# nubot-nudt/MDGAT-matcher

Hardware: AMD Instinct MI355X
Metric: keypoint-pairs/sec (higher is better)
Workload: dtype f32 (products as 3 split-f16 MFMAs, fp32 accumulate)

## Files before the change

mdgat_matcher_amd/csrc/sinkhorn.hip:

```cpp
#include "common.hpp"
#include <atomic>
#include <cstdlib>

namespace {

constexpr float NEG_BIG = -1.0e30f;

struct SkArgs {
    const float* scores;
    const float* alpha_dev;
    float alpha_host;
    float* Z;
    int N, M, iters;
    const unsigned* only_if;
    unsigned* status_fallback;
    const unsigned* pair_flags;
    const int* cnt0;
    const int* cnt1;
};

__device__ __forceinline__ float wave_max(float v) {
#pragma unroll
    for (int o = 32; o > 0; o >>= 1) v = fmaxf(v, __shfl_xor(v, o, 64));
    return v;
}
__device__ __forceinline__ float wave_sum(float v) {
#pragma unroll
    for (int o = 32; o > 0; o >>= 1) v += __shfl_xor(v, o, 64);
    return v;
}
__device__ __forceinline__ float ex2(float x) { return __builtin_amdgcn_exp2f(x); }
__device__ __forceinline__ float lg2(float x) { return __builtin_amdgcn_logf(x); }

__device__ __forceinline__ float wave_lse2(const float* x, int n, float extra, int lane) {
    float m = extra;
    for (int i = lane; i < n; i += 64) m = fmaxf(m, x[i]);
    m = wave_max(m);
    float s = 0.f;
    for (int i = lane; i < n; i += 64) s += ex2(x[i] - m);
    s = wave_sum(s) + ex2(extra - m);
    return m + lg2(s);
}

template <int NC, int NW, bool RAGGED = false>
__global__ __launch_bounds__(NW * 64) void sinkhorn_kernel(SkArgs a) {
    extern __shared__ __attribute__((aligned(16))) float smem[];
    const int Ns = a.N, Ms = a.M;
    int N = Ns, M = Ms;
    if constexpr (RAGGED) { N = __builtin_amdgcn_readfirstlane(a.cnt0[blockIdx.x]); M = __builtin_amdgcn_readfirstlane(a.cnt1[blockIdx.x]); }
    const int tid = threadIdx.x, lane = tid & 63;
    const int wave = __builtin_amdgcn_readfirstlane(tid >> 6);
    if (a.only_if) {
        const bool mine = (__hip_atomic_load(a.only_if, __ATOMIC_RELAXED, __HIP_MEMORY_SCOPE_AGENT) & 1u) != 0 ||
                          (a.pair_flags && __hip_atomic_load(a.pair_flags + blockIdx.x, __ATOMIC_RELAXED, __HIP_MEMORY_SCOPE_AGENT) != 0);
        if (!mine) return;
        if (tid == 0 && a.status_fallback) __hip_atomic_store(a.status_fallback, 1u, __ATOMIC_RELAXED, __HIP_MEMORY_SCOPE_SYSTEM);
    }
    const float* S = a.scores + (size_t)blockIdx.x * Ns * Ms;
    float* Z = a.Z + (size_t)blockIdx.x * (Ns + 1) * (Ms + 1);

    float* u = smem;
    float* v = u + (N + 1);
    float* pm = v + (M + 1);
    float* ps = pm + NW * M;

    const float alpha = (a.alpha_dev ? *a.alpha_dev : a.alpha_host) * MDGAT_LOG2E;
    const float norm = -logf((float)(N + M));
    const float lmu = norm * MDGAT_LOG2E;
    const float lmuN = (logf((float)M) + norm) * MDGAT_LOG2E;
    const float lnu = lmu;
    const float lnuM = (logf((float)N) + norm) * MDGAT_LOG2E;

    for (int i = tid; i <= N; i += NW * 64) u[i] = 0.f;
    for (int j = tid; j <= M; j += NW * 64) v[j] = 0.f;
    __syncthreads();

    for (int it = 0; it < a.iters; ++it) {
        float vr[NC];
#pragma unroll
        for (int c = 0; c < NC; ++c) {
            const int j = c * 64 + lane;
            vr[c] = j < M ? v[j] : 0.f;
        }
        const float bM = alpha + v[M];
        if (wave == NW - 1) {
            const float lse = alpha + wave_lse2(v, M, v[M], lane);
            if (lane == 0) u[N] = lmuN - lse;
        }
        float cm[NC], cs[NC];
#pragma unroll
        for (int c = 0; c < NC; ++c) { cm[c] = NEG_BIG; cs[c] = 0.f; }

        for (int i = wave; i < N; i += NW) {
            const float* row = S + (size_t)i * Ms;
            float s[NC];
#pragma unroll
            for (int c = 0; c < NC; ++c) {
                const int j = c * 64 + lane;
                s[c] = j < M ? row[j] * MDGAT_LOG2E : NEG_BIG;
            }
            float m = bM;
#pragma unroll
            for (int c = 0; c < NC; ++c) m = fmaxf(m, s[c] + vr[c]);
            m = wave_max(m);
            float e = 0.f;
#pragma unroll
            for (int c = 0; c < NC; ++c) e += ex2(s[c] + vr[c] - m);
            e = wave_sum(e) + ex2(bM - m);
            const float ui = lmu - (m + lg2(e));
            if (lane == 0) u[i] = ui;
#pragma unroll
            for (int c = 0; c < NC; ++c) {
                const float w = s[c] + ui;
                const float nm = fmaxf(cm[c], w);
                cs[c] = cs[c] * ex2(cm[c] - nm) + ex2(w - nm);
                cm[c] = nm;
            }
        }
#pragma unroll
        for (int c = 0; c < NC; ++c) {
            const int j = c * 64 + lane;
            if (j < M) { pm[wave * M + j] = cm[c]; ps[wave * M + j] = cs[c]; }
        }
        __syncthreads();
        const float bN = alpha + u[N];
        for (int j = tid; j < M; j += NW * 64) {
            float m = bN;
#pragma unroll
            for (int w = 0; w < NW; ++w) m = fmaxf(m, pm[w * M + j]);
            float e = ex2(bN - m);
#pragma unroll
            for (int w = 0; w < NW; ++w) e += ps[w * M + j] * ex2(pm[w * M + j] - m);
            v[j] = lnu - (m + lg2(e));
        }
        if (wave == 0) {
            const float lse = alpha + wave_lse2(u, N, u[N], lane);
            if (lane == 0) v[M] = lnuM - lse;
        }
        __syncthreads();
    }

    const float uN = u[N], vM = v[M];
    for (int i = wave; i < N; i += NW) {
        const float ui = u[i];
        const float* row = S + (size_t)i * Ms;
        float* zr = Z + (size_t)i * (Ms + 1);
        for (int j = lane; j < M; j += 64) zr[j] = (row[j] * MDGAT_LOG2E + ui + v[j]) * MDGAT_LN2 - norm;
        if (lane == 0) zr[M] = (alpha + ui + vM) * MDGAT_LN2 - norm;
        if constexpr (RAGGED)
            for (int j = M + 1 + lane; j <= Ms; j += 64) zr[j] = 0.f;
    }
    float* zl = Z + (size_t)N * (Ms + 1);
    for (int j = tid; j <= M; j += NW * 64) zl[j] = (alpha + uN + v[j]) * MDGAT_LN2 - norm;
    if constexpr (RAGGED) {
        float* rest = zl + M + 1;
        const int nrest = (Ms - M) + (Ns - N) * (Ms + 1);
        for (int j = tid; j < nrest; j += NW * 64) rest[j] = 0.f;
    }
}


constexpr int SLOT_STRIDE = 520;

template <int CTRL, int ROW_MASK>
__device__ __forceinline__ float dpp_move(float identity, float v) {
    return __builtin_bit_cast(float, __builtin_amdgcn_update_dpp(__builtin_bit_cast(int, identity), __builtin_bit_cast(int, v),
                                                                 CTRL, ROW_MASK, 0xf, false));
}
__device__ __forceinline__ float wave_max_dpp(float v) {
    v = fmaxf(v, dpp_move<0x111, 0xf>(NEG_BIG, v));
    v = fmaxf(v, dpp_move<0x112, 0xf>(NEG_BIG, v));
    v = fmaxf(v, dpp_move<0x114, 0xf>(NEG_BIG, v));
    v = fmaxf(v, dpp_move<0x118, 0xf>(NEG_BIG, v));
    v = fmaxf(v, dpp_move<0x142, 0xa>(NEG_BIG, v));
    v = fmaxf(v, dpp_move<0x143, 0xc>(NEG_BIG, v));
    return __builtin_bit_cast(float, __builtin_amdgcn_readlane(__builtin_bit_cast(int, v), 63));
}
__device__ __forceinline__ float wave_sum_dpp(float v) {
    v += dpp_move<0x111, 0xf>(0.f, v);
    v += dpp_move<0x112, 0xf>(0.f, v);
    v += dpp_move<0x114, 0xf>(0.f, v);
    v += dpp_move<0x118, 0xf>(0.f, v);
    v += dpp_move<0x142, 0xa>(0.f, v);
    v += dpp_move<0x143, 0xc>(0.f, v);
    return __builtin_bit_cast(float, __builtin_amdgcn_readlane(__builtin_bit_cast(int, v), 63));
}

__device__ __forceinline__ void swap_halves32(float& a, float& b) { asm("s_nop 1\n\tv_permlane32_swap_b32 %0, %1\n\ts_nop 1" : "+v"(a), "+v"(b)); }
__device__ __forceinline__ void swap_rows16(float& a, float& b) { asm("s_nop 1\n\tv_permlane16_swap_b32 %0, %1\n\ts_nop 1" : "+v"(a), "+v"(b)); }
template <int CTRL, int BANK>
__device__ __forceinline__ float dpp_bank_move(float old, float v) {
    return __builtin_bit_cast(float, __builtin_amdgcn_update_dpp(__builtin_bit_cast(int, old), __builtin_bit_cast(int, v), CTRL, 0xf, BANK, false));
}
__device__ __forceinline__ float wave_sum16(float (&acc)[16], int lane) {
    float s[8];
#pragma unroll
    for (int r = 0; r < 8; ++r) { float x = acc[r], y = acc[r + 8]; swap_halves32(x, y); s[r] = x + y; }
    float t[4];
#pragma unroll
    for (int r = 0; r < 4; ++r) { float x = s[r], y = s[r + 4]; swap_rows16(x, y); t[r] = x + y; }
    const bool b3 = (lane & 8) != 0, b2 = (lane & 4) != 0;
    float v[2];
#pragma unroll
    for (int r = 0; r < 2; ++r) {
        const float keep = b3 ? t[r + 2] : t[r], give = b3 ? t[r] : t[r + 2];
        v[r] = keep + dpp_bank_move<0x128, 0xf>(0.f, give);
    }
    const float keep = b2 ? v[1] : v[0], give = b2 ? v[0] : v[1];
    float o = dpp_bank_move<0x104, 0x5>(0.f, give);
    o = dpp_bank_move<0x114, 0xa>(o, give);
    float w = keep + o;
    w += dpp_bank_move<0xb1, 0xf>(0.f, w);
    w += dpp_bank_move<0x4e, 0xf>(0.f, w);
    return __builtin_bit_cast(float, __builtin_amdgcn_ds_bpermute(16 * lane, __builtin_bit_cast(int, w)));
}

typedef __attribute__((address_space(1))) unsigned long long gu64;
#define SK_LD "sc1"

struct SksArgs {
    const float* scores;
    const float* alpha_dev;
    float alpha_host;
    float* Z;
    unsigned long long* slots;
    unsigned* error_word;
    unsigned* pair_flags;
    unsigned* range_guard;
    int B, N, M, iters, ngroups, GR, GC;
    int xcd_map;
    int ext_mode;
    int* rbest_idx;
    float* rbest_val;
    int* cbest_idx;
    float* cbest_val;
};

constexpr int SKS_THREADS = 512;
constexpr int SKS_LDS_FLOATS = 520 + 8 * 512 + 8 + 8 + 8 * 512;
constexpr int ROW_STRIDE = 136;

__device__ __forceinline__ unsigned long long xload(gu64* p, bool same_xcd) {
    if (same_xcd) {
        unsigned long long v;
        asm volatile("global_load_dwordx2 %0, %1, off " SK_LD "\n\ts_waitcnt vmcnt(0)" : "=v"(v) : "v"(p) : "memory");
        return v;
    }
    return __hip_atomic_load(p, __ATOMIC_RELAXED, __HIP_MEMORY_SCOPE_AGENT);
}
__device__ __forceinline__ void xstore(gu64* p, unsigned long long v, bool same_xcd) {
    if (same_xcd) asm volatile("global_store_dwordx2 %0, %1, off" :: "v"(p), "v"(v) : "memory");
    else __hip_atomic_store(p, v, __ATOMIC_RELAXED, __HIP_MEMORY_SCOPE_AGENT);
}

template <int NMAX>
__device__ __forceinline__ void poll_partners(gu64* base, size_t stride, int n, int self, unsigned tag, float (&vals)[NMAX],
                                              bool& failed, unsigned* error_word, bool same_xcd = false,
                                              gu64* extra = nullptr, float* extra_val = nullptr) {
    unsigned pending = ((1u << n) - 1u) & ~(1u << self);
    bool extra_pending = extra != nullptr;
    unsigned spins = 0;
    while (pending || extra_pending) {
        unsigned long long x[NMAX], xe = 0;
        if (NMAX <= 4 && same_xcd) {
#pragma unroll
            for (int p = 0; p < NMAX; ++p)
                if (pending & (1u << p)) asm volatile("global_load_dwordx2 %0, %1, off " SK_LD : "=v"(x[p]) : "v"(base + (size_t)p * stride) : "memory");
            if (extra_pending) asm volatile("global_load_dwordx2 %0, %1, off " SK_LD : "=v"(xe) : "v"(extra) : "memory");
            asm volatile("s_waitcnt vmcnt(0)" ::: "memory");
#pragma unroll
            for (int p = 0; p < NMAX; ++p)
                if (pending & (1u << p)) asm volatile("" : "+v"(x[p]));
            asm volatile("" : "+v"(xe));
        } else if (same_xcd) {
#pragma unroll
            for (int p = 0; p < NMAX; ++p) x[p] = 0;
#pragma unroll
            for (int p0 = 0; p0 < NMAX; p0 += 4) {
                if (!((pending >> p0) & 0xfu) && !(extra_pending && p0 == 0)) continue;
                unsigned long long y[4] = {0, 0, 0, 0};
#pragma unroll
                for (int u = 0; u < 4; ++u)
                    if (pending & (1u << (p0 + u))) asm volatile("global_load_dwordx2 %0, %1, off " SK_LD : "=v"(y[u]) : "v"(base + (size_t)(p0 + u) * stride) : "memory");
                if (extra_pending && p0 == 0) asm volatile("global_load_dwordx2 %0, %1, off " SK_LD : "=v"(xe) : "v"(extra) : "memory");
                asm volatile("s_waitcnt vmcnt(0)" ::: "memory");
#pragma unroll
                for (int u = 0; u < 4; ++u) {
                    asm volatile("" : "+v"(y[u]));
                    if ((pending & (1u << (p0 + u))) && (unsigned)(y[u] >> 32) == tag) {
                        vals[p0 + u] = __builtin_bit_cast(float, (unsigned)y[u]);
                        pending &= ~(1u << (p0 + u));
                    }
                }
                asm volatile("" : "+v"(xe));
            }
        } else {
#pragma unroll
            for (int p = 0; p < NMAX; ++p)
                if (pending & (1u << p)) x[p] = __hip_atomic_load(base + (size_t)p * stride, __ATOMIC_RELAXED, __HIP_MEMORY_SCOPE_AGENT);
            if (extra_pending) xe = __hip_atomic_load(extra, __ATOMIC_RELAXED, __HIP_MEMORY_SCOPE_AGENT);
        }
#pragma unroll
        for (int p = 0; p < NMAX; ++p)
            if ((pending & (1u << p)) && (unsigned)(x[p] >> 32) == tag) {
                vals[p] = __builtin_bit_cast(float, (unsigned)x[p]);
                pending &= ~(1u << p);
            }
        if (extra_pending && (unsigned)(xe >> 32) == tag) {
            *extra_val = __builtin_bit_cast(float, (unsigned)xe);
            extra_pending = false;
        }
        if (pending || extra_pending) {
            if (failed || ++spins > (1u << 22)) { failed = true; atomicOr(error_word, 1u); break; }
            __builtin_amdgcn_s_sleep(1);
        }
    }
}

template <bool TWO_D, int GMAX>
__global__ __launch_bounds__(SKS_THREADS, 2) void sinkhorn_scaling_kernel(SksArgs a) {
    constexpr int RPW = 16;
    __shared__ __attribute__((aligned(16))) float lds[SKS_LDS_FLOATS];
    float* bvec = lds;
    float* colp = lds + 520;
    float* pdust = colp + 8 * 512;
    int* flags = reinterpret_cast<int*>(pdust + 8);
    int* colpi = flags + 8;

    const int N = a.N, M = a.M, GR = a.GR, GC = TWO_D ? a.GC : 1;
    const int tid = threadIdx.x, lane = tid & 63;
    const int wave = __builtin_amdgcn_readfirstlane(tid >> 6);
    const int P = GR * GC;
    int group, w;
    if (a.xcd_map) {
        const int xcd = blockIdx.x & 7, q = blockIdx.x >> 3;
        w = q % P;
        group = (q / P) * 8 + xcd;
        if (group >= a.ngroups) return;
    } else {
        group = blockIdx.x / P;
        w = blockIdx.x % P;
    }
    const int jr = w / GC, jc = w % GC;
    const float alpha = (a.alpha_dev ? *a.alpha_dev : a.alpha_host) * MDGAT_LOG2E;
    const float norm = -logf((float)(N + M));
    const float mu = 1.0f / (float)(N + M);
    const float muN = (float)M / (float)(N + M);
    const float nu = mu;
    const float nuM = (float)N / (float)(N + M);
    const int row0 = (jr * 8 + wave) * RPW;
    const int col0 = lane * 8;
    const int gcol0 = jc * 512 + col0;
    const bool my_row_valid = lane < RPW && row0 + lane < N;
    const size_t col_slots = (size_t)2 * GC * GR * SLOT_STRIDE, row_slots = (size_t)2 * GR * GC * ROW_STRIDE;
    gu64* cslots = (gu64*)(a.slots) + (size_t)group * (col_slots + row_slots);
    gu64* rslots = cslots + col_slots;
    unsigned cep = 0, rep_ = 0, xep = 0;
    bool failed = false;
    const float RANGE_HI = 1.099511627776e12f, RANGE_LO = 9.094947017729282e-13f;

    auto row_exchange = [&](float v, bool take_max) -> float {
        if (!TWO_D) return v;
        ++rep_;
        const bool active = lane <= RPW;
        const int idx = lane < RPW ? wave * RPW + lane : 128;
        float out = v;
        if (active) {
            gu64* base = rslots + ((size_t)(rep_ & 1) * GR + jr) * GC * ROW_STRIDE + idx;
            __hip_atomic_store(base + (size_t)jc * ROW_STRIDE, ((unsigned long long)rep_ << 32) | __builtin_bit_cast(unsigned, v),
                               __ATOMIC_RELAXED, __HIP_MEMORY_SCOPE_AGENT);
            float vals[4];
#pragma unroll
            for (int p = 0; p < 4; ++p) vals[p] = take_max ? NEG_BIG : 0.f;
            poll_partners<4>(base, ROW_STRIDE, GC, jc, rep_, vals, failed, a.error_word);
            out = take_max ? NEG_BIG : 0.f;
#pragma unroll
            for (int p = 0; p < 4; ++p) {
                const float x = (p == jc) ? v : vals[p];
                out = take_max ? fmaxf(out, x) : out + x;
            }
        }
        return out;
    };

    for (int pair = group; pair < a.B; pair += a.ngroups) {
        const float* S = a.scores + (size_t)pair * N * M;
        float K[RPW][8];
        const bool vec_ok = (M & 3) == 0 && gcol0 + 8 <= M;
        unsigned gmax = 0;
        if (vec_ok) {
#pragma unroll
            for (int r = 0; r < RPW; ++r) {
                const int i = row0 + r;
                const float* row = S + (size_t)min(i, N - 1) * M;
                const f32x4 x0 = *reinterpret_cast<const f32x4*>(row + gcol0);
                const f32x4 x1 = *reinterpret_cast<const f32x4*>(row + gcol0 + 4);
#pragma unroll
                for (int c = 0; c < 4; ++c) {
                    gmax = max(gmax, max(__builtin_bit_cast(unsigned, x0[c]) & 0x7fffffffu, __builtin_bit_cast(unsigned, x1[c]) & 0x7fffffffu));
                    K[r][c] = i < N ? x0[c] * MDGAT_LOG2E : NEG_BIG;
                    K[r][4 + c] = i < N ? x1[c] * MDGAT_LOG2E : NEG_BIG;
                }
            }
        } else if (gcol0 >= M) {
#pragma unroll
            for (int r = 0; r < RPW; ++r)
#pragma unroll
                for (int c = 0; c < 8; ++c) K[r][c] = NEG_BIG;
        } else {
#pragma unroll
            for (int r = 0; r < RPW; ++r) {
                const float* row = S + (size_t)min(row0 + r, N - 1) * M;
#pragma unroll
                for (int c = 0; c < 8; ++c) K[r][c] = row[min(gcol0 + c, M - 1)];
            }
#pragma unroll
            for (int r = 0; r < RPW; ++r)
#pragma unroll
                for (int c = 0; c < 8; ++c) {
                    const float x = K[r][c];
                    gmax = max(gmax, __builtin_bit_cast(unsigned, x) & 0x7fffffffu);
                    K[r][c] = (row0 + r < N && gcol0 + c < M) ? x * MDGAT_LOG2E : NEG_BIG;
                }
        }
        if (a.range_guard && gmax >= 0x7f800000u) __hip_atomic_store(a.range_guard, 1u, __ATOMIC_RELAXED, __HIP_MEMORY_SCOPE_SYSTEM);
        float u0r = 0.f, kbr = 0.f, ar = 0.f;
        {
            float mrow = NEG_BIG;
#pragma unroll
            for (int r = 0; r < RPW; ++r) {
                float m = K[r][0];
#pragma unroll
                for (int c = 1; c < 8; ++c) m = fmaxf(m, K[r][c]);
                m = wave_max_dpp(m);
                mrow = (lane == r) ? m : mrow;
            }
            mrow = fmaxf(row_exchange(mrow, true), alpha);
            u0r = -mrow;
#pragma unroll
            for (int r = 0; r < RPW; ++r) {
                const float m = __builtin_bit_cast(float, __builtin_amdgcn_readlane(__builtin_bit_cast(int, mrow), r));
#pragma unroll
                for (int c = 0; c < 8; ++c) K[r][c] = ex2(K[r][c] - m);
            }
        }
        if (my_row_valid) { kbr = ex2(alpha + u0r); ar = 1.f; } else { u0r = 0.f; }
        {
            float kmin = my_row_valid ? kbr : 1.f;
#pragma unroll
            for (int r = 0; r < RPW; ++r)
#pragma unroll
                for (int c = 0; c < 8; c += 2) {
                    const bool v0_ = row0 + r < N && gcol0 + c < M, v1_ = row0 + r < N && gcol0 + c + 1 < M;
                    kmin = fminf(kmin, fminf(v0_ ? K[r][c] : 1.f, v1_ ? K[r][c + 1] : 1.f));
                }
            if (kmin < 0x1p-100f) {
                atomicOr(a.error_word, 2u);
                __hip_atomic_store(a.pair_flags + pair, 1u, __ATOMIC_RELAXED, __HIP_MEMORY_SCOPE_AGENT);
            }
        }
        float u0N = -alpha, aN = 1.f;
        float v0[8], kr[8], b[8];
#pragma unroll
        for (int c = 0; c < 8; ++c) { v0[c] = 0.f; kr[c] = (gcol0 + c < M) ? 1.f : 0.f; b[c] = (gcol0 + c < M) ? 1.f : 0.f; }
        float v0M = 0.f, kc = 1.f, bM = 1.f;
        const bool tcol_valid = jc * 512 + tid < M;
        float krt = 1.f, v0t = 0.f, bt = 1.f;
        __syncthreads();
        if (tid == 0) flags[0] = 0;
        bool same_xcd = false;
        if (!TWO_D && GR > 1) {
            ++xep;
            if (tid == 0) {
                const unsigned my_xcc = __builtin_amdgcn_s_getreg((3 << 11) | 20) & 0xf;
                gu64* xb = cslots + (size_t)jc * GR * SLOT_STRIDE + 513;
                const unsigned xtag = 0x80000000u | xep;
                __hip_atomic_store(xb + (size_t)jr * SLOT_STRIDE, ((unsigned long long)xtag << 32) | my_xcc, __ATOMIC_RELAXED, __HIP_MEMORY_SCOPE_AGENT);
                float ids[GMAX];
#pragma unroll
                for (int pp = 0; pp < GMAX; ++pp) ids[pp] = 0.f;
                poll_partners<GMAX>(xb, SLOT_STRIDE, GR, jr, xtag, ids, failed, a.error_word);
                bool same = !failed;
#pragma unroll
                for (int pp = 0; pp < GMAX; ++pp)
                    if (pp < GR && pp != jr && __builtin_bit_cast(unsigned, ids[pp]) != my_xcc) same = false;
                flags[1] = same ? 1 : 0;
            }
            __syncthreads();
            same_xcd = flags[1] != 0;
        }

        for (int it = 0; it < a.iters; ++it) {
            float psum = 0.f;
            {
                float racc[16];
#pragma unroll
                for (int r = 0; r < 16; ++r) {
                    float acc = K[r][0] * b[0];
#pragma unroll
                    for (int c = 1; c < 8; ++c) acc = fmaf(K[r][c], b[c], acc);
                    racc[r] = acc;
                }
                psum = wave_sum16(racc, lane);
                psum = lane < 16 ? psum : 0.f;
            }
            {
                float pd = kr[0] * b[0];
#pragma unroll
                for (int c = 1; c < 8; ++c) pd = fmaf(kr[c], b[c], pd);
                pd = wave_sum_dpp(pd);
                if (TWO_D) {
                    psum = (lane == RPW) ? pd : psum;
                    psum = row_exchange(psum, false);
                    pd = __builtin_bit_cast(float, __builtin_amdgcn_readlane(__builtin_bit_cast(int, psum), RPW));
                }
                aN = muN * __builtin_amdgcn_rcpf(fmaf(kc, bM, pd));
            }
            ar = my_row_valid ? mu * __builtin_amdgcn_rcpf(fmaf(kbr, bM, psum)) : 0.f;
            const float dsum = wave_sum_dpp(kbr * ar);
            float q[8];
#pragma unroll
            for (int c = 0; c < 8; ++c) q[c] = 0.f;
#pragma unroll
            for (int r = 0; r < RPW; ++r) {
                const float arr = __builtin_bit_cast(float, __builtin_amdgcn_readlane(__builtin_bit_cast(int, ar), r));
#pragma unroll
                for (int c = 0; c < 8; ++c) q[c] = fmaf(K[r][c], arr, q[c]);
            }
            {
                f32x4* qw = reinterpret_cast<f32x4*>(colp + wave * 512 + col0);
                qw[0] = f32x4{q[0], q[1], q[2], q[3]};
                qw[1] = f32x4{q[4], q[5], q[6], q[7]};
                if (lane == 0) pdust[wave] = dsum;
            }
            __syncthreads();
            ++cep;
            {
                gu64* base = cslots + ((size_t)(cep & 1) * GC + jc) * GR * SLOT_STRIDE;
                const unsigned long long tagbits = (unsigned long long)cep << 32;
                float dloc = 0.f;
                if (wave == 7) {
                    dloc = pdust[0];
#pragma unroll
                    for (int ww = 1; ww < 8; ++ww) dloc += pdust[ww];
                    if (GR > 1 && lane == 0) xstore(base + (size_t)jr * SLOT_STRIDE + 512, tagbits | __builtin_bit_cast(unsigned, dloc), same_xcd);
                }
                bool have_dust = false;
                float dust_in = 0.f;
                if (tcol_valid) {
                    float loc = colp[tid];
#pragma unroll
                    for (int ww = 1; ww < 8; ++ww) loc += colp[ww * 512 + tid];
                    float vals[GMAX];
#pragma unroll
                    for (int pp = 0; pp < GMAX; ++pp) vals[pp] = 0.f;
                    if (GR > 1) {
                        xstore(base + (size_t)jr * SLOT_STRIDE + tid, tagbits | __builtin_bit_cast(unsigned, loc), same_xcd);
                        const bool my_dust = wave == 7 && lane < GR && lane != jr;
                        poll_partners<GMAX>(base + tid, SLOT_STRIDE, GR, jr, cep, vals, failed, a.error_word, same_xcd,
                                            my_dust ? base + (size_t)lane * SLOT_STRIDE + 512 : nullptr, &dust_in);
                        have_dust = my_dust && !failed;
                    }
                    float total = 0.f;
#pragma unroll
                    for (int pp = 0; pp < GMAX; ++pp) total += (pp == jr) ? loc : vals[pp];
                    bt = nu * __builtin_amdgcn_rcpf(fmaf(krt, aN, total));
                    bvec[tid] = bt;
                    if (!(bt > RANGE_LO && bt < RANGE_HI)) flags[0] = 1;
                }
                if (wave == 7) {
                    float mine = have_dust ? dust_in : dloc;
                    if (GR > 1) {
                        if (lane < GR && lane != jr && !have_dust) {
                            unsigned spins = 0;
                            while (true) {
                                const unsigned long long x = xload(base + (size_t)lane * SLOT_STRIDE + 512, same_xcd);
                                if ((unsigned)(x >> 32) == cep) { mine = __builtin_bit_cast(float, (unsigned)x); break; }
                                if (failed || ++spins > (1u << 22)) { failed = true; atomicOr(a.error_word, 1u); break; }
                                __builtin_amdgcn_s_sleep(1);
                            }
                        }
                    }
                    float total = 0.f;
#pragma unroll
                    for (int pp = 0; pp < GMAX; ++pp)
                        if (pp < GR) total += __builtin_bit_cast(float, __builtin_amdgcn_readlane(__builtin_bit_cast(int, mine), pp));
                    if (lane == 0) bvec[512] = nuM * __builtin_amdgcn_rcpf(fmaf(kc, aN, total));
                }
            }
            __syncthreads();
            {
                const f32x4 x0 = *reinterpret_cast<const f32x4*>(bvec + col0);
                const f32x4 x1 = *reinterpret_cast<const f32x4*>(bvec + col0 + 4);
                b[0] = x0[0]; b[1] = x0[1]; b[2] = x0[2]; b[3] = x0[3]; b[4] = x1[0]; b[5] = x1[1]; b[6] = x1[2]; b[7] = x1[3];
#pragma unroll
                for (int c = 0; c < 8; ++c) if (gcol0 + c >= M) b[c] = 0.f;
                bM = bvec[512];
            }
            if (flags[0] != 0) {
#pragma unroll
                for (int c = 0; c < 8; ++c) {
                    if (gcol0 + c < M) {
#pragma unroll
                        for (int r = 0; r < RPW; ++r) K[r][c] *= b[c];
                        v0[c] += lg2(b[c]);
                        kr[c] *= b[c];
                        b[c] = 1.f;
                    }
                }
                if (tcol_valid) { krt *= bt; v0t += lg2(bt); bt = 1.f; }
                __syncthreads();
                if (tid == 0) flags[0] = 0;
            }
            if (!(bM > RANGE_LO && bM < RANGE_HI)) {
                kbr *= bM;
                kc *= bM;
                v0M += lg2(bM);
                bM = 1.f;
            }
            if (!(aN > RANGE_LO && aN < RANGE_HI)) {
#pragma unroll
                for (int c = 0; c < 8; ++c) kr[c] *= aN;
                krt *= aN;
                kc *= aN;
                u0N += lg2(aN);
                aN = 1.f;
            }
            {
                const bool fold = my_row_valid && !(ar > RANGE_LO && ar < RANGE_HI);
                const unsigned long long fm = __ballot(fold);
                if (fm) {
#pragma unroll
                    for (int r = 0; r < RPW; ++r) {
                        if (fm & (1ull << r)) {
                            const float arr = __builtin_bit_cast(float, __builtin_amdgcn_readlane(__builtin_bit_cast(int, ar), r));
#pragma unroll
                            for (int c = 0; c < 8; ++c) K[r][c] *= arr;
                        }
                    }
                    if (fold) { kbr *= ar; u0r += lg2(ar); ar = 1.f; }
                }
            }
        }

        float* Zp = a.Z ? a.Z + (size_t)pair * (N + 1) * (M + 1) : nullptr;
        const bool partner_lost = (__hip_atomic_load(a.error_word, __ATOMIC_RELAXED, __HIP_MEMORY_SCOPE_AGENT) & 1u) != 0 ||
                                  __hip_atomic_load(a.pair_flags + pair, __ATOMIC_RELAXED, __HIP_MEMORY_SCOPE_AGENT) != 0;
        const float poison = partner_lost ? __builtin_nanf("") : 0.f;
        const bool ran = a.iters > 0;
        const float VM = ran ? v0M + lg2(bM) + poison : 0.f;
        const float Ur = (ran && my_row_valid) ? u0r + lg2(ar) : 0.f;
        float V[8];
#pragma unroll
        for (int c = 0; c < 8; ++c) V[c] = (ran && gcol0 + c < M) ? v0[c] + lg2(b[c]) : 0.f;
        constexpr bool FROM_K = !TWO_D && GMAX == 4;
        const float dUr = Ur - u0r;
        float dV[8];
#pragma unroll
        for (int c = 0; c < 8; ++c) dV[c] = V[c] - v0[c];
        const bool ext = a.ext_mode >= 0;
        const bool inner = a.ext_mode >= MDGAT_EXTRACT_THRESHOLD;
        const bool last_c = jc == GC - 1, last_r = jr == GR - 1;
        float cbv[8];
        int cbi[8];
#pragma unroll
        for (int c = 0; c < 8; ++c) { cbv[c] = -__builtin_inff(); cbi[c] = 0; }
#pragma unroll
        for (int r = 0; r < RPW; ++r) {
            const int i = row0 + r;
            if (i < N) {
                const float U = __builtin_bit_cast(float, __builtin_amdgcn_readlane(__builtin_bit_cast(int, Ur), r));
                const float dU = __builtin_bit_cast(float, __builtin_amdgcn_readlane(__builtin_bit_cast(int, dUr), r));
                const float* row = S + (size_t)i * M;
                float z[8];
                if (FROM_K) {
                    bool under = false;
#pragma unroll
                    for (int c = 0; c < 8; ++c) {
                        under |= (gcol0 + c < M) && !(K[r][c] >= 1.17549435e-38f);
                        z[c] = (gcol0 + c < M) ? (lg2(K[r][c]) + dU + dV[c]) * MDGAT_LN2 - norm : -__builtin_inff();
                    }
                    if (__any(under)) {
#pragma unroll
                        for (int c = 0; c < 8; ++c)
                            if ((gcol0 + c < M) && !(K[r][c] >= 1.17549435e-38f)) z[c] = (row[gcol0 + c] * MDGAT_LOG2E + U + V[c]) * MDGAT_LN2 - norm;
                    }
                } else {
#pragma unroll
                    for (int c = 0; c < 8; ++c)
                        z[c] = (gcol0 + c < M) ? (row[min(gcol0 + c, M - 1)] * MDGAT_LOG2E + U + V[c]) * MDGAT_LN2 - norm : -__builtin_inff();
                }
                const float zM = (alpha + U + VM) * MDGAT_LN2 - norm;
                if (Zp) {
                    float* zr = Zp + (size_t)i * (M + 1);
#pragma unroll
                    for (int c = 0; c < 8; ++c)
                        if (gcol0 + c < M) zr[gcol0 + c] = z[c];
                    if (last_c && lane == 0) zr[M] = zM;
                }
                if (ext) {
                    float bv = z[0];
                    int bi = gcol0;
#pragma unroll
                    for (int c = 1; c < 8; ++c)
                        if (z[c] > bv) { bv = z[c]; bi = gcol0 + c; }
                    {
                        const float mx = wave_max_dpp(bv);
                        const unsigned long long hit = __ballot(bv == mx);
                        const int first = hit ? __builtin_ctzll(hit) : 0;
                        bi = __builtin_amdgcn_readlane(bi, first);
                        bv = __builtin_bit_cast(float, __builtin_amdgcn_readlane(__builtin_bit_cast(int, bv), first));
                    }
                    if (!inner && last_c && zM > bv) { bv = zM; bi = M; }
                    if (lane == 0) {
                        a.rbest_idx[((size_t)pair * GC + jc) * N + i] = bi;
                        a.rbest_val[((size_t)pair * GC + jc) * N + i] = bv;
                    }
#pragma unroll
                    for (int c = 0; c < 8; ++c)
                        if (z[c] > cbv[c]) { cbv[c] = z[c]; cbi[c] = i; }
                }
            }
        }
        const float UN = ran ? u0N + lg2(aN) : 0.f;
        const float zNt = (alpha + UN + (ran ? v0t + lg2(bt) + poison : 0.f)) * MDGAT_LN2 - norm;
        if (last_r && Zp) {
            float* zl = Zp + (size_t)N * (M + 1);
            if (tcol_valid) zl[jc * 512 + tid] = zNt;
            if (last_c && tid == 0) zl[M] = (alpha + UN + VM) * MDGAT_LN2 - norm;
        }
        if (ext) {
            __syncthreads();
            {
                f32x4* qw = reinterpret_cast<f32x4*>(colp + wave * 512 + col0);
                qw[0] = f32x4{cbv[0], cbv[1], cbv[2], cbv[3]};
                qw[1] = f32x4{cbv[4], cbv[5], cbv[6], cbv[7]};
                int* qi = colpi + wave * 512 + col0;
#pragma unroll
                for (int c = 0; c < 8; ++c) qi[c] = cbi[c];
            }
            __syncthreads();
            if (tcol_valid) {
                float bv = colp[tid];
                int bi = colpi[tid];
#pragma unroll
                for (int ww = 1; ww < 8; ++ww) {
                    const float v = colp[ww * 512 + tid];
                    if (v > bv) { bv = v; bi = colpi[ww * 512 + tid]; }
                }
                if (!inner && last_r && zNt > bv) { bv = zNt; bi = N; }
                a.cbest_val[((size_t)pair * GR + jr) * M + jc * 512 + tid] = bv;
                a.cbest_idx[((size_t)pair * GR + jr) * M + jc * 512 + tid] = bi;
            }
        }
    }
}

struct ExArgs {
    const float* Z;
    int N, M, mode;
    float thr;
    int64_t* m0; int64_t* m1;
    float* s0; float* s1;
    const unsigned* sk_error;
    const float* Zfb;
    const unsigned* pair_flags;
    unsigned* alldust_counters;
    int B;
    const int* rbest_idx; const float* rbest_val; const int* cbest_idx; const float* cbest_val; int GR, GC;
    unsigned* matched; unsigned matched_token;
    const int* cnt0; const int* cnt1;
};

__global__ __launch_bounds__(1024) void extract_kernel(ExArgs a) {
    extern __shared__ __attribute__((aligned(16))) float smem[];
    const int Ns = a.N, Ms = a.M;
    int N = Ns, M = Ms;
    if (a.cnt0) { N = a.cnt0[blockIdx.x]; M = a.cnt1[blockIdx.x]; }
    const int tid = threadIdx.x, lane = tid & 63, wave = tid >> 6;
    const bool redone = a.sk_error && ((__hip_atomic_load(a.sk_error, __ATOMIC_RELAXED, __HIP_MEMORY_SCOPE_AGENT) & 1u) != 0 ||
                                       (a.pair_flags && __hip_atomic_load(a.pair_flags + blockIdx.x, __ATOMIC_RELAXED, __HIP_MEMORY_SCOPE_AGENT) != 0));
    const float* Zsrc = redone ? a.Zfb : a.Z;
    const float* Z = Zsrc + (size_t)blockIdx.x * (Ns + 1) * (Ms + 1);
    int* idx0 = reinterpret_cast<int*>(smem);
    int* idx1 = idx0 + Ns;
    float* val0 = reinterpret_cast<float*>(idx1 + Ms);
    float* val1 = val0 + Ns;
    const bool inner = a.mode >= MDGAT_EXTRACT_THRESHOLD;
    const int ncol = inner ? M : M + 1;
    const int nrow = inner ? N : N + 1;
    if (!Zsrc) {
        for (int i = tid; i < N; i += 1024) {
            const size_t base = (size_t)blockIdx.x * a.GC * Ns + i;
            float bv = a.rbest_val[base];
            int bi = a.rbest_idx[base];
            for (int g = 1; g < a.GC; ++g) {
                const float v = a.rbest_val[base + (size_t)g * Ns];
                if (v > bv) { bv = v; bi = a.rbest_idx[base + (size_t)g * Ns]; }
            }
            idx0[i] = bi; val0[i] = bv;
        }
        for (int j = tid; j < M; j += 1024) {
            const size_t base = (size_t)blockIdx.x * a.GR * Ms + j;
            float bv = a.cbest_val[base];
            int bi = a.cbest_idx[base];
            for (int g = 1; g < a.GR; ++g) {
                const float v = a.cbest_val[base + (size_t)g * Ms];
                if (v > bv) { bv = v; bi = a.cbest_idx[base + (size_t)g * Ms]; }
            }
            idx1[j] = bi; val1[j] = bv;
        }
    } else {
    for (int i = wave; i < N; i += 16) {
        const float* zr = Z + (size_t)i * (Ms + 1);
        float bv = -__builtin_inff();
        int bi = 0x7fffffff;
        for (int j = lane; j < ncol; j += 64) {
            const float z = zr[j];
            if (z > bv) { bv = z; bi = j; }
        }
#pragma unroll
        for (int o = 32; o > 0; o >>= 1) {
            const float ov = __shfl_xor(bv, o, 64);
            const int oi = __shfl_xor(bi, o, 64);
            if (ov > bv || (ov == bv && oi < bi)) { bv = ov; bi = oi; }
        }
        if (lane == 0) { idx0[i] = bi; val0[i] = bv; }
    }
    for (int j = tid; j < M; j += 1024) {
        float bv = -__builtin_inff();
        int bi = 0;
        for (int i = 0; i < nrow; ++i) {
            const float z = Z[(size_t)i * (Ms + 1) + j];
            if (z > bv) { bv = z; bi = i; }
        }
        idx1[j] = bi; val1[j] = bv;
    }
    }
    __syncthreads();

    int64_t* m0 = a.m0 + (size_t)blockIdx.x * Ns;
    int64_t* m1 = a.m1 + (size_t)blockIdx.x * Ms;
    float* s0 = a.s0 + (size_t)blockIdx.x * Ns;
    float* s1 = a.s1 + (size_t)blockIdx.x * Ms;

    int nmatch = 0;
    if (a.mode == MDGAT_EXTRACT_DUSTBIN || a.mode == MDGAT_EXTRACT_DUSTBIN_MUTUAL) {
        const bool mutual = a.mode == MDGAT_EXTRACT_DUSTBIN_MUTUAL;
        int nvalid = 0;
        for (int i = tid; i < N; i += 1024) {
            const int j = idx0[i];
            const bool valid = j < M;
            const bool keep = valid && (!mutual || idx1[j] == i);
            m0[i] = valid ? j : -1;
            s0[i] = keep ? expf(val0[i]) : 0.f;
            nvalid += valid;
        }
        for (int j = tid; j < M; j += 1024) {
            const int i = idx1[j];
            const bool valid = i < N;
            const bool keep = valid && (!mutual || idx0[i] == j);
            m1[j] = valid ? i : -1;
            s1[j] = keep ? expf(val1[j]) : 0.f;
        }
        nmatch = nvalid;
        if (a.alldust_counters) {
            const int any_valid = __syncthreads_or(nvalid > 0);
            __shared__ int last;
            if (tid == 0) {
                __threadfence();
                const unsigned old = atomicAdd(a.alldust_counters, (any_valid ? 0x10000u : 0u) + 1u);
                last = (old & 0xffffu) == (unsigned)a.B - 1 && (old >> 16) == 0 && !any_valid;
                __threadfence();
            }
            __syncthreads();
            if (last) {
                float* s1all = a.s1;
                for (size_t i = tid; i < (size_t)a.B * Ms; i += 1024) s1all[i] = 0.f;
            }
        } else if (a.cnt0) {
            if (!__syncthreads_or(nvalid > 0))
                for (int j = tid; j < M; j += 1024) s1[j] = 0.f;
        }
    } else if (a.mode == MDGAT_EXTRACT_THRESHOLD) {
        for (int i = tid; i < N; i += 1024) {
            const float e = expf(val0[i]);
            const bool valid = e > a.thr;
            m0[i] = valid ? idx0[i] : -1;
            s0[i] = valid ? e : 0.f;
            nmatch += valid;
        }
        for (int j = tid; j < M; j += 1024) {
            const float e = expf(val1[j]);
            const bool valid = e > a.thr;
            m1[j] = valid ? idx1[j] : -1;
            s1[j] = valid ? e : 0.f;
        }
    } else {
        for (int i = tid; i < N; i += 1024) {
            const bool mutual0 = idx1[idx0[i]] == i;
            const float ms0 = mutual0 ? expf(val0[i]) : 0.f;
            const bool valid0 = mutual0 && ms0 > a.thr;
            m0[i] = valid0 ? idx0[i] : -1;
            s0[i] = ms0;
            nmatch += valid0;
        }
        for (int j = tid; j < M; j += 1024) {
            const int i = idx1[j];
            const bool mutual1 = idx0[i] == j;
            const bool mutual0_i = idx1[idx0[i]] == i;
            const float ms0_i = mutual0_i ? expf(val0[i]) : 0.f;
            const float ms1 = mutual1 ? ms0_i : 0.f;
            const bool valid1 = mutual1 && (mutual0_i && ms0_i > a.thr);
            m1[j] = valid1 ? i : -1;
            s1[j] = ms1;
        }
    }
    if (a.cnt0) {
        for (int i = N + tid; i < Ns; i += 1024) { m0[i] = -1; s0[i] = 0.f; }
        for (int j = M + tid; j < Ms; j += 1024) { m1[j] = -1; s1[j] = 0.f; }
    }
    if (a.matched) {
        const int any = __syncthreads_or(nmatch > 0);
        if (any && tid == 0) __hip_atomic_store(a.matched, a.matched_token, __ATOMIC_RELAXED, __HIP_MEMORY_SCOPE_SYSTEM);
    }
}

__global__ __launch_bounds__(256) void extract_alldust_fixup(const int64_t* m0, size_t n0, float* s1, size_t n1) {
    for (size_t base = 0; base < n0; base += 256) {
        const size_t i = base + threadIdx.x;
        if (__syncthreads_or(i < n0 && m0[i] >= 0)) return;
    }
    for (size_t i = blockIdx.x * (size_t)256 + threadIdx.x; i < n1; i += (size_t)gridDim.x * 256) s1[i] = 0.f;
}

template <int NC, int NW, bool RAGGED = false>
int launch_sk(const SkArgs& a, int B, hipStream_t s) {
    const size_t lds = ((size_t)(a.N + 1) + (a.M + 1) + 2 * (size_t)NW * a.M) * sizeof(float);
    hipError_t e = hipFuncSetAttribute(reinterpret_cast<const void*>(sinkhorn_kernel<NC, NW, RAGGED>),
                                       hipFuncAttributeMaxDynamicSharedMemorySize, (int)lds);
    if (e != hipSuccess) return mdgat_check_hip(e, "sinkhorn LDS attribute");
    hipLaunchKernelGGL((sinkhorn_kernel<NC, NW, RAGGED>), dim3(B), dim3(NW * 64), lds, s, a);
    return mdgat_check_hip(hipGetLastError(), "sinkhorn launch");
}

}

static void sk_tiling(int N, int M, int& GR, int& GC) { GR = (N + 127) / 128; GC = (M + 511) / 512; }
static int sk_max_groups(int N, int M) {
    int GR, GC;
    sk_tiling(N, M, GR, GC);
    int g = 256 / (GR * GC);
    return g > 64 ? 64 : (g < 1 ? 1 : g);
}
static size_t slots_bytes(int N, int M) {
    int GR, GC;
    sk_tiling(N, M, GR, GC);
    const size_t per_group = ((size_t)2 * GC * GR * SLOT_STRIDE + (size_t)2 * GR * GC * ROW_STRIDE) * sizeof(unsigned long long);
    return (256 + per_group * sk_max_groups(N, M) + 255) & ~(size_t)255;
}
static size_t flags_bytes(int B) { return ((size_t)B * sizeof(unsigned) + 255) & ~(size_t)255; }
size_t sinkhorn_cluster_workspace_bytes(int B, int N, int M) {
    if (N > 2048 || M > 2048) return 0;
    int GR, GC;
    sk_tiling(N, M, GR, GC);
    return slots_bytes(N, M) + flags_bytes(B) + ((size_t)B * GC * N * 2 + (size_t)B * GR * M * 2) * sizeof(float);
}

static int launch_extract_impl(int B, int N, int M, ExArgs a, hipStream_t s, bool defer_alldust = false);

static std::atomic<unsigned long long> sinkhorn_launch_count[SK_COUNTERS];
static void sinkhorn_count_launch(int index) { sinkhorn_launch_count[index].fetch_add(1, std::memory_order_relaxed); }
void sinkhorn_launch_counts(uint64_t counts[MDGAT_SINKHORN_COUNTERS]) {
    for (int i = 0; i < SK_COUNTERS; ++i) counts[i] = sinkhorn_launch_count[i].load(std::memory_order_relaxed);
}

bool sinkhorn_workspace_usable(int B, int N, int M, const void* ws, size_t ws_bytes) {
    const size_t need = sinkhorn_cluster_workspace_bytes(B, N, M);
    return need && ws && ws_bytes >= need && (reinterpret_cast<uintptr_t>(ws) & 255) == 0;
}

SkPlan sinkhorn_plan(int B, int N, int M, int num_cu, bool workspace, bool fallback_buffer, bool ragged) {
    SkPlan p{SK_PATH_NONE, -1, -1, 0, 0, 0, 0, 0, 0, MDGAT_OK};
    if (B <= 0 || N <= 0 || M <= 0) return p;
    const int nc = M <= 64 ? 0 : M <= 128 ? 1 : M <= 256 ? 2 : M <= 512 ? 3 : (M <= 1024 && N <= 4096) ? 4 : (M <= 2048 && N <= 4096) ? 5 : -1;
    if (ragged) {
        if (N > MDGAT_RAGGED_FP32_MAX_KEYPOINTS || M > MDGAT_RAGGED_FP32_MAX_KEYPOINTS) { p.rc = MDGAT_ERR_UNSUPPORTED; return p; }
        p.path = SK_PATH_STREAMING;
        p.stream = SK_RAGGED_1 + nc;
        p.grid = B;
        return p;
    }
    if (!workspace || N > 2048 || M > 2048) {
        if (nc < 0) { p.rc = MDGAT_ERR_UNSUPPORTED; return p; }
        p.path = SK_PATH_STREAMING;
        p.stream = SK_STREAM_1 + nc;
        p.grid = B;
        return p;
    }
    sk_tiling(N, M, p.GR, p.GC);
    const int P = p.GR * p.GC;
    int ngroups = num_cu / P;
    if (ngroups > sk_max_groups(N, M)) ngroups = sk_max_groups(N, M);
    if (ngroups > B) ngroups = B;
    p.ngroups = ngroups;
    if (ngroups < 1) { p.rc = MDGAT_ERR_UNSUPPORTED; return p; }
    const int ng8 = (ngroups + 7) & ~7;
    p.xcd_map = P * (ng8 / 8) <= num_cu / 8;
    p.grid = p.xcd_map ? ng8 * P : ngroups * P;
    p.path = SK_PATH_CLUSTER;
    p.scaling = p.GC > 1 ? SK_SCALING_2D : p.GR > 4 ? SK_SCALING_16 : SK_SCALING_4;
    const bool can_fall_back = fallback_buffer && nc >= 0;
    p.cooperative = !can_fall_back || ngroups * P > num_cu;
    if (can_fall_back) p.stream = SK_STREAM_1 + nc;
    return p;
}

static int launch_streaming(const SkArgs& a, int B, int form, bool gated, hipStream_t s) {
    int rc;
    switch (form) {
    case SK_STREAM_1: rc = launch_sk<1, 16>(a, B, s); break;
    case SK_STREAM_2: rc = launch_sk<2, 16>(a, B, s); break;
    case SK_STREAM_4: rc = launch_sk<4, 16>(a, B, s); break;
    case SK_STREAM_8: rc = launch_sk<8, 16>(a, B, s); break;
    case SK_STREAM_16: rc = launch_sk<16, 8>(a, B, s); break;
    case SK_STREAM_32: rc = launch_sk<32, 8>(a, B, s); break;
    case SK_RAGGED_1: rc = launch_sk<1, 16, true>(a, B, s); break;
    case SK_RAGGED_2: rc = launch_sk<2, 16, true>(a, B, s); break;
    case SK_RAGGED_4: rc = launch_sk<4, 16, true>(a, B, s); break;
    case SK_RAGGED_8: rc = launch_sk<8, 16, true>(a, B, s); break;
    default:
        mdgat_set_error("sinkhorn: M=%d > 2048 unsupported", a.M);
        return MDGAT_ERR_UNSUPPORTED;
    }
    if (!rc) sinkhorn_count_launch(gated ? SK_GATED : form);
    return rc;
}

int launch_sinkhorn_ragged(int B, int N, int M, const int* cnt0, const int* cnt1, const float* scores, const float* bin_score_dev, float bin_score_host,
                           int iters, float* Z, const SkExtract* ex, hipStream_t s) {
    if (B <= 0) return MDGAT_OK;
    if (!cnt0 || !cnt1 || !scores || !Z) { mdgat_set_error("sinkhorn (ragged): null pointer"); return MDGAT_ERR_BAD_ARG; }
    if (N <= 0 || M <= 0 || iters < 0) { mdgat_set_error("sinkhorn (ragged): bad shape N=%d M=%d iters=%d", N, M, iters); return MDGAT_ERR_BAD_ARG; }
    const SkPlan p = sinkhorn_plan(B, N, M, 0, false, true, true);
    if (p.rc) {
        mdgat_set_error("sinkhorn (ragged): padded sizes %d x %d: at most %d keypoints per frame", N, M, MDGAT_RAGGED_FP32_MAX_KEYPOINTS);
        return p.rc;
    }
    const SkArgs a{scores, bin_score_dev, bin_score_host, Z, N, M, iters, nullptr, nullptr, nullptr, cnt0, cnt1};
    const int rc = launch_streaming(a, B, p.stream, false, s);
    if (rc || !ex) return rc;
    ExArgs xa{Z, N, M, ex->mode, ex->thr, ex->m0, ex->m1, ex->s0, ex->s1, nullptr, nullptr, nullptr, nullptr, B, nullptr, nullptr, nullptr, nullptr, 1, 1,
              ex->matched, ex->matched_token, cnt0, cnt1};
    return launch_extract_impl(B, N, M, xa, s, ex->defer_alldust != 0);
}

size_t sinkhorn_slots_clear_bytes(int B, int N, int M) { return (N > 2048 || M > 2048) ? 0 : slots_bytes(N, M) + flags_bytes(B); }

static int launch_scaling(const SkPlan& pl, int B, int N, int M, const float* scores, const float* alpha_dev, float alpha_host, int iters,
                          float* Z, void* ws, const SkExtract* ex, unsigned* status, float* Zfb, bool slots_cleared, hipStream_t s) {
    const int GR = pl.GR, GC = pl.GC, ngroups = pl.ngroups;
    if (pl.rc) { mdgat_set_error("sinkhorn: %d workgroups per pair do not fit the device", GR * GC); return pl.rc; }
    const size_t per_group = ((size_t)2 * GC * GR * SLOT_STRIDE + (size_t)2 * GR * GC * ROW_STRIDE) * sizeof(unsigned long long);
    if (!slots_cleared) {
        if (int rc = mdgat_check_hip(hipMemsetAsync(ws, 0, 256 + per_group * ngroups, s), "memset(sinkhorn slots)")) return rc;
        if (int rc = mdgat_check_hip(hipMemsetAsync(static_cast<char*>(ws) + slots_bytes(N, M), 0, flags_bytes(B), s), "memset(sinkhorn pair flags)")) return rc;
    }
    if (const char* f = getenv("MDGAT_SK_FORCE_FALLBACK"); f && *f == '1')
        if (int rc = mdgat_check_hip(hipMemsetAsync(ws, 1, sizeof(unsigned), s), "memset(sinkhorn error word)")) return rc;
    SksArgs a{scores, alpha_dev, alpha_host, Z, reinterpret_cast<unsigned long long*>(static_cast<char*>(ws) + 256),
              static_cast<unsigned*>(ws), reinterpret_cast<unsigned*>(static_cast<char*>(ws) + slots_bytes(N, M)),
              status ? status + MDGAT_STATUS_RANGE : nullptr, B, N, M, iters, ngroups, GR, GC, pl.xcd_map, -1, nullptr, nullptr, nullptr, nullptr};
    if (ex) {
        char* p = static_cast<char*>(ws) + slots_bytes(N, M) + flags_bytes(B);
        a.ext_mode = ex->mode;
        a.rbest_idx = reinterpret_cast<int*>(p);                      p += (size_t)B * GC * N * sizeof(int);
        a.rbest_val = reinterpret_cast<float*>(p);                    p += (size_t)B * GC * N * sizeof(float);
        a.cbest_idx = reinterpret_cast<int*>(p);                      p += (size_t)B * GR * M * sizeof(int);
        a.cbest_val = reinterpret_cast<float*>(p);
    }
    void* args[] = {&a};
    const void* kern = pl.scaling == SK_SCALING_2D ? reinterpret_cast<const void*>(sinkhorn_scaling_kernel<true, 16>)
                     : pl.scaling == SK_SCALING_16 ? reinterpret_cast<const void*>(sinkhorn_scaling_kernel<false, 16>)
                                                  : reinterpret_cast<const void*>(sinkhorn_scaling_kernel<false, 4>);
    float* zfb = Z ? Z : Zfb;
    const bool can_fall_back = pl.stream >= 0;
    hipError_t e;
    if (pl.cooperative) e = hipLaunchCooperativeKernel(kern, dim3(pl.grid), dim3(SKS_THREADS), args, 0, s);
    else e = hipLaunchKernel(kern, dim3(pl.grid), dim3(SKS_THREADS), args, 0, s);
    if (int rc = mdgat_check_hip(e, "sinkhorn scaling launch")) return rc;
    sinkhorn_count_launch(pl.scaling);
    if (can_fall_back) {
        SkArgs f{scores, alpha_dev, alpha_host, zfb, N, M, iters, a.error_word, status ? status + MDGAT_STATUS_SK_FALLBACK : nullptr, a.pair_flags};
        if (int rc = launch_streaming(f, B, pl.stream, true, s)) return rc;
    }
    if (ex) {
        ExArgs x{nullptr, N, M, ex->mode, ex->thr, ex->m0, ex->m1, ex->s0, ex->s1, can_fall_back ? a.error_word : nullptr, zfb, a.pair_flags,
                 (ex->defer_alldust || B >= 65536) ? nullptr : a.error_word + 2, B,
                 a.rbest_idx, a.rbest_val, a.cbest_idx, a.cbest_val, GR, GC, ex->matched, ex->matched_token};
        return launch_extract_impl(B, N, M, x, s, ex->defer_alldust != 0);
    }
    return MDGAT_OK;
}

size_t mdgat_sinkhorn_ws_bytes_impl(int B, int N, int M) { return sinkhorn_cluster_workspace_bytes(B, N, M); }

int launch_sinkhorn(int B, int N, int M, const float* scores, const float* bin_score_dev, float bin_score_host,
                    int iters, float* Z, void* ws, size_t ws_bytes, const SkExtract* ex, hipStream_t s, unsigned* status, float* Zfb,
                    bool slots_cleared) {
    if (B <= 0) return MDGAT_OK;
    if (!Z && !ex) { mdgat_set_error("sinkhorn: nothing to compute (no Z, no extraction)"); return MDGAT_ERR_BAD_ARG; }
    if (N <= 0 || M <= 0 || iters < 0) { mdgat_set_error("sinkhorn: bad shape N=%d M=%d iters=%d", N, M, iters); return MDGAT_ERR_BAD_ARG; }
    const bool usable = sinkhorn_workspace_usable(B, N, M, ws, ws_bytes);
    const SkPlan p = sinkhorn_plan(B, N, M, usable ? mdgat_cu_count() : 0, usable, Z || Zfb, false);
    if (usable) return launch_scaling(p, B, N, M, scores, bin_score_dev, bin_score_host, iters, Z, ws, ex, status, Zfb, slots_cleared, s);
    if (!Z) { mdgat_set_error("sinkhorn: the streaming kernel needs a Z buffer"); return MDGAT_ERR_BAD_ARG; }
    SkArgs a{scores, bin_score_dev, bin_score_host, Z, N, M, iters, nullptr, nullptr, nullptr};
    const int rc = launch_streaming(a, B, p.stream, false, s);
    if (rc || !ex) return rc;
    ExArgs xa{Z, N, M, ex->mode, ex->thr, ex->m0, ex->m1, ex->s0, ex->s1, nullptr, nullptr, nullptr, nullptr, B, nullptr, nullptr, nullptr, nullptr, 1, 1,
              ex->matched, ex->matched_token};
    return launch_extract_impl(B, N, M, xa, s, ex->defer_alldust != 0);
}

int launch_alldust_fixup(int B, int N, int M, int mode, const int64_t* m0, float* s1, hipStream_t s) {
    if (mode != MDGAT_EXTRACT_DUSTBIN && mode != MDGAT_EXTRACT_DUSTBIN_MUTUAL) return MDGAT_OK;
    const size_t n = (size_t)B * M;
    hipLaunchKernelGGL(extract_alldust_fixup, dim3((unsigned)((n + 255) / 256 < 16 ? (n + 255) / 256 : 16)), dim3(256), 0, s,
                       m0, (size_t)B * N, s1, n);
    return mdgat_check_hip(hipGetLastError(), "extract fixup launch");
}

static int launch_extract_impl(int B, int N, int M, ExArgs a, hipStream_t s, bool defer_alldust) {
    if (a.mode < 0 || a.mode > 3) { mdgat_set_error("extract: bad mode %d", a.mode); return MDGAT_ERR_BAD_ARG; }
    const size_t lds = (size_t)(2 * (N + M) + 4) * sizeof(float);
    hipLaunchKernelGGL(extract_kernel, dim3(B), dim3(1024), lds, s, a);
    if (int rc = mdgat_check_hip(hipGetLastError(), "extract launch")) return rc;
    sinkhorn_count_launch(SK_EXTRACT);
    if (defer_alldust || a.alldust_counters || a.cnt0) return MDGAT_OK;
    return launch_alldust_fixup(B, N, M, a.mode, a.m0, a.s1, s);
}

int launch_extract_from_bests(int B, int N, int M, const SkExtract* ex, const int* rbest_idx, const float* rbest_val, const int* cbest_idx,
                              const float* cbest_val, hipStream_t s, const int* cnt0, const int* cnt1) {
    if (B <= 0) return MDGAT_OK;
    if ((cnt0 != nullptr) != (cnt1 != nullptr)) { mdgat_set_error("extract: per-pair counts for one frame only"); return MDGAT_ERR_BAD_ARG; }
    ExArgs xa{nullptr, N, M, ex->mode, ex->thr, ex->m0, ex->m1, ex->s0, ex->s1, nullptr, nullptr, nullptr, nullptr, B, rbest_idx, rbest_val, cbest_idx, cbest_val,
              1, 1, ex->matched, ex->matched_token, cnt0, cnt1};
    return launch_extract_impl(B, N, M, xa, s, ex->defer_alldust != 0);
}

int launch_extract(int B, int N, int M, const float* Z, int mode, float thr, int64_t* m0, int64_t* m1, float* s0,
                   float* s1, hipStream_t s) {
    if (B <= 0) return MDGAT_OK;
    ExArgs a{Z, N, M, mode, thr, m0, m1, s0, s1, nullptr, nullptr, nullptr, nullptr, B, nullptr, nullptr, nullptr, nullptr, 1, 1, nullptr, 0u};
    return launch_extract_impl(B, N, M, a, s);
}
```

Baseline: 21320.

## Park column log-scale offsets in LDS and batch permlane swaps in row reduction

For the 1-D GMAX==4 variant, the per-column log offsets (v0[8], v0t, v0M) move out of registers into an extra LDS array. They are updated there during range folds and reloaded only after the iteration loop, which lowers register pressure in the hot loop. The wave_sum16 reduction also gains a grouped mode that issues all permlane32/permlane16 swaps in one asm block with a single pair of s_nops instead of one pair per swap. The costs are a little more LDS per block and an extra syncthreads before the epilogue.

```diff
diff --git a/mdgat_matcher_amd/csrc/sinkhorn.hip b/mdgat_matcher_amd/csrc/sinkhorn.hip
--- a/mdgat_matcher_amd/csrc/sinkhorn.hip
+++ b/mdgat_matcher_amd/csrc/sinkhorn.hip
@@ -188,17 +188,44 @@
 
 __device__ __forceinline__ void swap_halves32(float& a, float& b) { asm("s_nop 1\n\tv_permlane32_swap_b32 %0, %1\n\ts_nop 1" : "+v"(a), "+v"(b)); }
 __device__ __forceinline__ void swap_rows16(float& a, float& b) { asm("s_nop 1\n\tv_permlane16_swap_b32 %0, %1\n\ts_nop 1" : "+v"(a), "+v"(b)); }
+__device__ __forceinline__ void swap_halves32x8(float (&a)[8], float (&b)[8]) {
+    asm("s_nop 1\n\t"
+        "v_permlane32_swap_b32 %0, %8\n\tv_permlane32_swap_b32 %1, %9\n\tv_permlane32_swap_b32 %2, %10\n\tv_permlane32_swap_b32 %3, %11\n\t"
+        "v_permlane32_swap_b32 %4, %12\n\tv_permlane32_swap_b32 %5, %13\n\tv_permlane32_swap_b32 %6, %14\n\tv_permlane32_swap_b32 %7, %15\n\t"
+        "s_nop 1"
+        : "+v"(a[0]), "+v"(a[1]), "+v"(a[2]), "+v"(a[3]), "+v"(a[4]), "+v"(a[5]), "+v"(a[6]), "+v"(a[7]),
+          "+v"(b[0]), "+v"(b[1]), "+v"(b[2]), "+v"(b[3]), "+v"(b[4]), "+v"(b[5]), "+v"(b[6]), "+v"(b[7]));
+}
+__device__ __forceinline__ void swap_rows16x4(float (&a)[4], float (&b)[4]) {
+    asm("s_nop 1\n\t"
+        "v_permlane16_swap_b32 %0, %4\n\tv_permlane16_swap_b32 %1, %5\n\tv_permlane16_swap_b32 %2, %6\n\tv_permlane16_swap_b32 %3, %7\n\t"
+        "s_nop 1"
+        : "+v"(a[0]), "+v"(a[1]), "+v"(a[2]), "+v"(a[3]), "+v"(b[0]), "+v"(b[1]), "+v"(b[2]), "+v"(b[3]));
+}
 template <int CTRL, int BANK>
 __device__ __forceinline__ float dpp_bank_move(float old, float v) {
     return __builtin_bit_cast(float, __builtin_amdgcn_update_dpp(__builtin_bit_cast(int, old), __builtin_bit_cast(int, v), CTRL, 0xf, BANK, false));
 }
+template <bool GROUPED>
 __device__ __forceinline__ float wave_sum16(float (&acc)[16], int lane) {
-    float s[8];
-#pragma unroll
-    for (int r = 0; r < 8; ++r) { float x = acc[r], y = acc[r + 8]; swap_halves32(x, y); s[r] = x + y; }
-    float t[4];
-#pragma unroll
-    for (int r = 0; r < 4; ++r) { float x = s[r], y = s[r + 4]; swap_rows16(x, y); t[r] = x + y; }
+    float x8[8], y8[8], s[8];
+#pragma unroll
+    for (int r = 0; r < 8; ++r) { x8[r] = acc[r]; y8[r] = acc[r + 8]; }
+    if (GROUPED) swap_halves32x8(x8, y8);
+#pragma unroll
+    for (int r = 0; r < 8; ++r) {
+        if (!GROUPED) swap_halves32(x8[r], y8[r]);
+        s[r] = x8[r] + y8[r];
+    }
+    float x4[4], y4[4], t[4];
+#pragma unroll
+    for (int r = 0; r < 4; ++r) { x4[r] = s[r]; y4[r] = s[r + 4]; }
+    if (GROUPED) swap_rows16x4(x4, y4);
+#pragma unroll
+    for (int r = 0; r < 4; ++r) {
+        if (!GROUPED) swap_rows16(x4[r], y4[r]);
+        t[r] = x4[r] + y4[r];
+    }
     const bool b3 = (lane & 8) != 0, b2 = (lane & 4) != 0;
     float v[2];
 #pragma unroll
@@ -238,6 +265,7 @@
 
 constexpr int SKS_THREADS = 512;
 constexpr int SKS_LDS_FLOATS = 520 + 8 * 512 + 8 + 8 + 8 * 512;
+constexpr int SKS_PARK_FLOATS = 520;
 constexpr int ROW_STRIDE = 136;
 
 __device__ __forceinline__ unsigned long long xload(gu64* p, bool same_xcd) {
@@ -320,12 +348,14 @@
 template <bool TWO_D, int GMAX>
 __global__ __launch_bounds__(SKS_THREADS, 2) void sinkhorn_scaling_kernel(SksArgs a) {
     constexpr int RPW = 16;
-    __shared__ __attribute__((aligned(16))) float lds[SKS_LDS_FLOATS];
+    constexpr bool PARK = !TWO_D && GMAX == 4;
+    __shared__ __attribute__((aligned(16))) float lds[SKS_LDS_FLOATS + (PARK ? SKS_PARK_FLOATS : 0)];
     float* bvec = lds;
     float* colp = lds + 520;
     float* pdust = colp + 8 * 512;
     int* flags = reinterpret_cast<int*>(pdust + 8);
     int* colpi = flags + 8;
+    float* v0s = reinterpret_cast<float*>(colpi + 8 * 512);
 
     const int N = a.N, M = a.M, GR = a.GR, GC = TWO_D ? a.GC : 1;
     const int tid = threadIdx.x, lane = tid & 63;
@@ -468,6 +498,10 @@
         float krt = 1.f, v0t = 0.f, bt = 1.f;
         __syncthreads();
         if (tid == 0) flags[0] = 0;
+        if (PARK) {
+            v0s[tid] = 0.f;
+            if (tid == 0) v0s[512] = 0.f;
+        }
         bool same_xcd = false;
         if (!TWO_D && GR > 1) {
             ++xep;
@@ -501,7 +535,7 @@
                     for (int c = 1; c < 8; ++c) acc = fmaf(K[r][c], b[c], acc);
                     racc[r] = acc;
                 }
-                psum = wave_sum16(racc, lane);
+                psum = wave_sum16<!TWO_D>(racc, lane);
                 psum = lane < 16 ? psum : 0.f;
             }
             {
@@ -603,19 +637,24 @@
                     if (gcol0 + c < M) {
 #pragma unroll
                         for (int r = 0; r < RPW; ++r) K[r][c] *= b[c];
-                        v0[c] += lg2(b[c]);
+                        if (!PARK) v0[c] += lg2(b[c]);
                         kr[c] *= b[c];
                         b[c] = 1.f;
                     }
                 }
-                if (tcol_valid) { krt *= bt; v0t += lg2(bt); bt = 1.f; }
+                if (tcol_valid) {
+                    krt *= bt;
+                    if (PARK) v0s[tid] += lg2(bt); else v0t += lg2(bt);
+                    bt = 1.f;
+                }
                 __syncthreads();
                 if (tid == 0) flags[0] = 0;
             }
             if (!(bM > RANGE_LO && bM < RANGE_HI)) {
                 kbr *= bM;
                 kc *= bM;
-                v0M += lg2(bM);
+                if (!PARK) v0M += lg2(bM);
+                else if (tid == 0) v0s[512] += lg2(bM);
                 bM = 1.f;
             }
             if (!(aN > RANGE_LO && aN < RANGE_HI)) {
@@ -648,6 +687,14 @@
                                   __hip_atomic_load(a.pair_flags + pair, __ATOMIC_RELAXED, __HIP_MEMORY_SCOPE_AGENT) != 0;
         const float poison = partner_lost ? __builtin_nanf("") : 0.f;
         const bool ran = a.iters > 0;
+        if (PARK) {
+            __syncthreads();
+            const f32x4 x0 = *reinterpret_cast<const f32x4*>(v0s + col0);
+            const f32x4 x1 = *reinterpret_cast<const f32x4*>(v0s + col0 + 4);
+            v0[0] = x0[0]; v0[1] = x0[1]; v0[2] = x0[2]; v0[3] = x0[3]; v0[4] = x1[0]; v0[5] = x1[1]; v0[6] = x1[2]; v0[7] = x1[3];
+            v0t = v0s[tid];
+            v0M = v0s[512];
+        }
         const float VM = ran ? v0M + lg2(bM) + poison : 0.f;
         const float Ur = (ran && my_row_valid) ? u0r + lg2(ar) : 0.f;
         float V[8];
```

Measured after the change: 21330 (median of 4 runs). Within noise of the previous version (+0.0%).
